# chahuja/mix-stage

Hardware: AMD Instinct MI355X
Metric: train-step clips/sec (B=32, T=64, M=8) (higher is better)
Workload: dtype f32; 1 GPU; Mix-StAGE GAN train step (reference D/G coin flip, seed 4321: 457 G + 510 D steps), B=32 clips per GPU, T=64, 128-mel, 104-dim pose, M=S=8, audio branch pinned; fp32 arithmetic (the reference trains in fp64, trainer.py:138; held to it at 1e-4 pose L1); global_batch=32, parallelism=dp1, hip_graphs=True, bn_sync=local

## Files before the change

### include/mixstage_aux.h

```cpp
#ifndef MIXSTAGE_AUX_H_
#define MIXSTAGE_AUX_H_

#include "mixstage.h"

#ifdef __cplusplus
extern "C" {
#endif

int ms_set_counter_buffer(int32_t* zeroed_counters, int n);

int ms_conv_block_bwd_overlap(const ms_conv_desc* d, const float* x, const float* x2, const float* w,
                              const float* gamma, const float* running_mean, const float* running_var,
                              const float* y_raw, const float* y, const float* save, const float* dy, float* dyr,
                              float* dx, float* dx2, float* dw, float* dbias, float* dgamma, float* dbeta,
                              void* workspace, size_t workspace_bytes, void* stream, void* side_stream,
                              void* side_workspace, size_t side_workspace_bytes);

int ms_timing_enable(int on);
size_t ms_timing_report(char* buf, size_t cap);

int ms_debug_set_patch_min_workgroups(int n);
int ms_debug_set_patch_tuning(int intra_split, int force_splitk);

int ms_debug_set_conv16_tile(int wm, int wn);
int ms_debug_set_conv16_ring(int nstg, int wide8);
int ms_debug_set_wgrad16_target(int workgroups);
int ms_debug_set_wgrad16_ring(int buffers);
int ms_debug_set_wgrad_target(int workgroups);
int ms_debug_set_wgrad_wave(int on);
int ms_debug_set_conv_tile(int on);
int ms_debug_set_bn_fused(int on);
int ms_debug_set_bn_fused_min_workgroups(int n);
int ms_debug_set_skip(const char* patterns);

int ms_debug_set_clip32(int on);

int ms_debug_set_clip_corun(int on);
int ms_debug_set_clip_corun_bwd(int on);

int ms_selftest_mfma(const float* A, const float* B, float* C, int K, void* stream);
int ms_probe_peak(int kind, long iters, void* a, void* b, double* work, void* stream);

#ifdef __cplusplus
}
#endif
#endif
```

### mix_stage_amd/_lib.py

```python
import ctypes
import os

_HERE = os.path.dirname(os.path.abspath(__file__))
LIB_PATH = os.path.join(_HERE, 'libmixstage_hip.so')
_ALT_LIB = os.environ.get('MS_LIB_PATH')
if _ALT_LIB:
  LIB_PATH = _ALT_LIB

c_void_p, c_int, c_float, c_size_t = ctypes.c_void_p, ctypes.c_int, ctypes.c_float, ctypes.c_size_t


class BwdOptions(ctypes.Structure):
  _fields_ = [('side_stream', ctypes.c_void_p), ('side_workspace', ctypes.c_void_p), ('side_workspace_bytes', ctypes.c_size_t),
              ('wt_prepared', ctypes.c_void_p), ('wgrad_partials', ctypes.c_void_p), ('defer_wgrad_launch', ctypes.c_int),
              ('prev_y', ctypes.c_void_p), ('prev_y_raw', ctypes.c_void_p), ('prev_save', ctypes.c_void_p), ('prev_gamma', ctypes.c_void_p),
              ('prev_dgamma', ctypes.c_void_p), ('prev_dbeta', ctypes.c_void_p), ('prev_dbias', ctypes.c_void_p), ('prev_slope', ctypes.c_float),
              ('bn_sync', ctypes.c_void_p), ('bn_sync_words', ctypes.c_int32), ('dy_is_dyr', ctypes.c_int),
              ('dx_accum', ctypes.c_void_p)]


class LossScale(ctypes.Structure):
  _fields_ = [('scale', ctypes.c_float), ('scale_dev', ctypes.c_void_p)]


# ... 142 lines not shown
    'ms_debug_set_patch_min_workgroups': (c_int, [c_int]),
    'ms_debug_set_patch_tuning': (c_int, [c_int, c_int]),
    'ms_debug_set_conv16_tile': (c_int, [c_int, c_int]),
    'ms_debug_set_conv16_ring': (c_int, [c_int, c_int]),
    'ms_debug_set_skip': (c_int, [ctypes.c_char_p]),
    'ms_debug_set_clip32': (c_int, [c_int]),
    'ms_debug_set_clip_corun': (c_int, [c_int]),
    'ms_clip_hold': (c_int, [_P]),
    'ms_clip_hold_flush': (c_int, [_P]),
    'ms_clip_hold_discard': (c_int, [_P]),
    'ms_clip_grid': (c_int, [_DESC]),
    'ms_clip_pair_ok': (c_int, [_DESC, _DESC]),
    'ms_clip_dgrad_grid': (c_int, [_DESC]),
    'ms_clip_dgrad_pair_ok': (c_int, [_DESC, _DESC]),
    'ms_debug_set_clip_corun_bwd': (c_int, [c_int]),
    'ms_debug_set_wgrad16_target': (c_int, [c_int]),
    'ms_debug_set_wgrad16_ring': (c_int, [c_int]),
    'ms_debug_set_wgrad_target': (c_int, [c_int]),
    'ms_debug_set_wgrad_wave': (c_int, [c_int]),
    'ms_debug_set_conv_tile': (c_int, [c_int]),
    'ms_set_wgrad_batched': (c_int, [c_int, c_int]),
    'ms_dgrad_fuses_prev_bn': (c_int, [_P]),
    'ms_dgrad_takes_accum': (c_int, [_P]),
    'ms_stat_pair_ok': (c_int, [_P]),
    'ms_selftest_mfma': (c_int, [_P, _P, _P, c_int, _P]),
    'ms_probe_peak': (c_int, [c_int, ctypes.c_long, _P, _P, ctypes.POINTER(ctypes.c_double), _P]),
}

_lib = None

# ... 42 lines not shown
```

### mix_stage_amd/csrc/api.hip

```cpp
#include "block_geom.h"

namespace ms {
extern int g_clip32;

static int validate(const ms_conv_desc* d, const char* who) {
  if (!d) return set_error("%s: null descriptor", who);
  if (d->B < 1 || d->Cin < 1 || d->Cout < 1 || d->groups < 1 || d->H < 1 || d->W < 1 || d->KH < 1 || d->KW < 1 ||
      d->SH < 1 || d->SW < 1 || d->PH < 0 || d->PW < 0)
    return set_error("%s: bad geometry", who);
  const int oh = (d->H + 2 * d->PH - d->KH) / d->SH + 1, ow = (d->W + 2 * d->PW - d->KW) / d->SW + 1;
  if (d->H + 2 * d->PH < d->KH || d->W + 2 * d->PW < d->KW || oh != d->OH || ow != d->OW)
    return set_error("%s: output size (%d,%d) does not match geometry (expected %d,%d)", who, d->OH, d->OW, oh, ow);
  if (d->mode < MS_BARE || d->mode > MS_BN_EVAL) return set_error("%s: bad mode %d", who, d->mode);
  if (d->in_mode < MS_IN_PLAIN || d->in_mode > MS_IN_UP2ADD) return set_error("%s: bad in_mode %d", who, d->in_mode);
  if (d->in_mode == MS_IN_UP2ADD && (d->H != 1 || d->KH != 1 || (d->W & 1)))
    return set_error("%s: UP2ADD needs a 1-D block with even W", who);
  if (dt_of(d) > DT_F16 || (d->dtype & ~(0xff | MS_DT_OUT_F32 | MS_DT_BN_FOLDED | MS_DT_STAT_PAIR | MS_DT_BN_FROZEN))) return set_error("%s: bad dtype 0x%x", who, d->dtype);
  if (dt_of(d) == DT_F32 && (d->dtype & ~(0xff | MS_DT_STAT_PAIR | MS_DT_BN_FROZEN))) return set_error("%s: MS_DT_OUT_F32 is a flag of the 16-bit modes", who);
  if ((d->dtype & MS_DT_BN_FROZEN) && d->mode != MS_BN_EVAL) return set_error("%s: MS_DT_BN_FROZEN is a flag of BN_EVAL blocks", who);
  if ((d->dtype & MS_DT_STAT_PAIR) && (d->B & 1)) return set_error("%s: MS_DT_STAT_PAIR needs an even batch", who);
  const double out_elems = (double)d->B * d->groups * d->Cout * d->OH * d->OW;
  const double in_elems = (double)d->B * d->groups * d->Cin * d->H * d->W;
  const double lim = dt_of(d) == DT_F32 ? 536870912.0 : 1073741824.0;
  if (out_elems >= lim || in_elems >= lim) return set_error("%s: tensor of 2 GiB or more (%.0f elements)", who, std::max(out_elems, in_elems));
// ... 742 lines not shown
}
int ms_clip_dgrad_pair_ok(const ms_conv_desc* host, const ms_conv_desc* guest) {
  if (validate(host, "ms_clip_dgrad_pair_ok") || validate(guest, "ms_clip_dgrad_pair_ok") || dt_of(host) != DT_F32 || dt_of(guest) != DT_F32 || g_precision != 0) return 0;
  return clip32_dgrad_pair_ok(host, guest) ? 1 : 0;
}
int ms_debug_set_clip_corun(int on) {
  const int prev = g_clip_corun < 0 ? 1 : g_clip_corun;
  g_clip_corun = on ? 1 : 0;
  return prev;
}
int ms_debug_set_clip_corun_bwd(int on) {
  const int prev = g_clip_corun_bwd < 0 ? 1 : g_clip_corun_bwd;
  g_clip_corun_bwd = on ? 1 : 0;
  return prev;
}

}
```

### mix_stage_amd/csrc/clip32.hip

```cpp
#include <stdio.h>
#include <stdlib.h>

#include <algorithm>
#include <map>
#include <mutex>
#include <vector>

#include "kernels.h"
#include "conv16.h"
#include "job_queue.h"

namespace ms {

typedef unsigned int cl_u32x4 __attribute__((ext_vector_type(4)));
typedef unsigned int cl_u32x2 __attribute__((ext_vector_type(2)));
constexpr int CL_SPIN_LIMIT = 1 << 21;
constexpr int CL_MAXK8W = 9;

struct Clip32Args {
  const float* x;
  const float* x2;
  const float* wp;
  const float* bias;
  const float* gamma;
// ... 721 lines not shown
    case 8: return clip32_launch_k<KW, S, NB, UP2, 8, DG2>(a, nwg, lds_bytes, s);
    case 9: return clip32_launch_k<KW, S, NB, UP2, 9, DG2>(a, nwg, lds_bytes, s);
    default: return clip32_launch_k<KW, S, NB, UP2, 0, DG2>(a, nwg, lds_bytes, s);
  }
}

struct ClipJob {
  Clip32Args a;
  int KW, S, nb, nwg, lds;
  bool up2, dg2;
  bool bwd;
  const char* what;
  double flops, bytes;
};

enum { CLIP_HOST_DOWN8 = 0, CLIP_HOST_UP8 = 1, CLIP_HOSTS = 2 };
enum { CLIP_GUEST_K3_4 = 0, CLIP_GUEST_DOWN2 = 1, CLIP_GUEST_DOWN4 = 2, CLIP_GUEST_DOWN8 = 3, CLIP_GUESTS = 4 };
enum { CLIP_BHOST_UP8 = 0, CLIP_BHOST_DOWN8 = 1 };
enum { CLIP_BGUEST_DG0 = 0, CLIP_BGUEST_DG2 = 1, CLIP_BGUEST_DG4 = 2, CLIP_BGUEST_DG8 = 3 };
static int clip_host_kind(const ClipJob& j) {
  if (j.a.k8w != 8) return -1;
  if (j.bwd) {
    if (j.up2) return -1;
    return j.dg2 ? CLIP_BHOST_DOWN8 : (j.KW == 3 && j.S == 1) ? CLIP_BHOST_UP8 : -1;
  }
  if (j.dg2) return -1;
  if (j.KW == 4 && j.S == 2 && !j.up2) return CLIP_HOST_DOWN8;
  if (j.KW == 3 && j.S == 1 && j.up2) return CLIP_HOST_UP8;
  return -1;
}
static int clip_guest_kind(const ClipJob& j) {
  if (j.up2) return -1;
  if (j.bwd) {
    if (!j.dg2) return -1;
    return j.a.k8w == 2 ? CLIP_BGUEST_DG2 : j.a.k8w == 4 ? CLIP_BGUEST_DG4 : j.a.k8w == 8 ? CLIP_BGUEST_DG8 : j.a.k8w == 9 ? -1 : CLIP_BGUEST_DG0;
  }
  if (j.dg2) return -1;
  if (j.KW == 3 && j.S == 1) return j.a.k8w == 4 ? CLIP_GUEST_K3_4 : -1;
  if (j.KW == 4 && j.S == 2) return j.a.k8w == 2 ? CLIP_GUEST_DOWN2 : j.a.k8w == 4 ? CLIP_GUEST_DOWN4 : j.a.k8w == 8 ? CLIP_GUEST_DOWN8 : -1;
  return -1;
}
static bool clip_pair_instance(const ClipJob& A, const ClipJob& B) {
  const int h = clip_host_kind(A), g = clip_guest_kind(B);
  if (h < 0 || g < 0 || A.bwd != B.bwd) return false;
  if (!A.bwd) return true;
  return h == CLIP_BHOST_UP8 ? (g == CLIP_BGUEST_DG0 || g == CLIP_BGUEST_DG8) : g != CLIP_BGUEST_DG0;
}
template <int KWA, int SA, int NBA, bool UP2A, int K8WA, int KWB, int SB, int NBB, bool UP2B, int K8WB, bool DG2A = false, bool DG2B = false>
static int clip32_pair_launch_k(const ClipPairArgs& pp, int nwg, int lds_bytes, hipStream_t s) {
  auto fn = clip32_pair_kernel<KWA, SA, NBA, UP2A, K8WA, KWB, SB, NBB, UP2B, K8WB, DG2A, DG2B>;
  static unsigned long long attr_done = 0;
  if (first_time_on_device(attr_done)) {
    if (hipFuncSetAttribute(reinterpret_cast<const void*>(fn), hipFuncAttributeMaxDynamicSharedMemorySize, 160 * 1024) != hipSuccess)
      return set_error("clip32: cannot raise the dynamic LDS limit");
    done_on_device(attr_done);
  }
  hipLaunchKernelGGL(fn, dim3(nwg), dim3(256), lds_bytes, s, pp);
  return check_launch("clip32_pair_kernel");
}
template <int KWA, int SA, int NBA, bool UP2A>
static int clip32_pair_launch_g(int guest, const ClipPairArgs& pp, int nwg, int lds_bytes, hipStream_t s) {
  switch (guest) {
    case CLIP_GUEST_K3_4: return clip32_pair_launch_k<KWA, SA, NBA, UP2A, 8, 3, 1, 2, false, 4>(pp, nwg, lds_bytes, s);
    case CLIP_GUEST_DOWN2: return clip32_pair_launch_k<KWA, SA, NBA, UP2A, 8, 4, 2, 1, false, 2>(pp, nwg, lds_bytes, s);
    case CLIP_GUEST_DOWN4: return clip32_pair_launch_k<KWA, SA, NBA, UP2A, 8, 4, 2, 1, false, 4>(pp, nwg, lds_bytes, s);
    default: return clip32_pair_launch_k<KWA, SA, NBA, UP2A, 8, 4, 2, 1, false, 8>(pp, nwg, lds_bytes, s);
  }
}
static int clip32_pair_launch_bwd(int host, int guest, const ClipPairArgs& pp, int nwg, int lds_bytes, hipStream_t s) {
  if (host == CLIP_BHOST_UP8) {
    if (guest == CLIP_BGUEST_DG0) return clip32_pair_launch_k<3, 1, 2, false, 8, 4, 1, 2, false, 0, false, true>(pp, nwg, lds_bytes, s);
    return clip32_pair_launch_k<3, 1, 2, false, 8, 4, 1, 2, false, 8, false, true>(pp, nwg, lds_bytes, s);
  }
  switch (guest) {
    case CLIP_BGUEST_DG2: return clip32_pair_launch_k<4, 1, 2, false, 8, 4, 1, 2, false, 2, true, true>(pp, nwg, lds_bytes, s);
    case CLIP_BGUEST_DG4: return clip32_pair_launch_k<4, 1, 2, false, 8, 4, 1, 2, false, 4, true, true>(pp, nwg, lds_bytes, s);
    default: return clip32_pair_launch_k<4, 1, 2, false, 8, 4, 1, 2, false, 8, true, true>(pp, nwg, lds_bytes, s);
  }
}

static int clip32_issue(ClipJob& j, hipStream_t s) {
  Clip32Args& a = j.a;
  const int nwg = j.nwg;
  TimingScope ts(s, j.flops, j.bytes, "clip32_kernel<%d,%d,%d,%d>|conv_%s_clip k1x%d s%d rows%d red%d T%d B%d ep%d", j.KW, j.S, j.nb, j.up2 ? 1 : 0, j.what,
// ... 21 lines not shown
      for (int k = 0; k < 8; ++k) {
        std::vector<double> v;
        for (int i = 0; i < nwg; ++i) if (h[(size_t)i * 8 + k]) v.push_back((double)(h[(size_t)i * 8 + k] - t0) * 0.01);
        if (v.empty()) continue;
        std::sort(v.begin(), v.end());
        fprintf(stderr, "  stamp %d: %7.2f %7.2f %7.2f\n", k, v.front(), v[v.size() / 2], v.back());
      }
    }
    a.stamps = nullptr;
  }
  return rc;
}

int g_clip_corun = -1;
int g_clip_corun_bwd = -1;
enum { HOLD_IDLE = 0, HOLD_ARMED = 1, HOLD_PENDING = 2 };
struct ClipHold {
  int state = HOLD_IDLE;
  ClipJob job;
  const char* ws_lo = nullptr;
  const char* ws_hi = nullptr;
};
static std::mutex g_hold_mu;
static std::map<hipStream_t, ClipHold> g_hold;
static thread_local bool t_in_call = false;
static thread_local const char* t_ws_lo = nullptr;
static thread_local const char* t_ws_hi = nullptr;

static bool clip_corun_on() {
  if (g_clip_corun < 0) { const char* e = getenv("MS_CLIP_CORUN"); g_clip_corun = e ? (atoi(e) != 0) : 1; }
  return g_clip_corun != 0;
}
static bool clip_corun_bwd_on() {
  if (g_clip_corun_bwd < 0) { const char* e = getenv("MS_CLIP_CORUN_BWD"); g_clip_corun_bwd = e ? (atoi(e) != 0) : 1; }
  return g_clip_corun_bwd != 0;
}

int clip32_hold_arm(hipStream_t s) {
  std::lock_guard<std::mutex> lk(g_hold_mu);
  ClipHold& h = g_hold[s];
  if (h.state == HOLD_PENDING) return set_error("ms_clip_hold: a held block is pending on this stream (flush or discard it first)");
  h.state = HOLD_ARMED;
  return 0;
}
void clip32_hold_discard(hipStream_t s) {
  std::lock_guard<std::mutex> lk(g_hold_mu);
  auto it = g_hold.find(s);
  if (it != g_hold.end()) it->second.state = HOLD_IDLE;
}
int clip32_hold_flush(hipStream_t s) {
  ClipJob job;
  {
// ... 41 lines not shown
  if (meetA && meetB && (A.a.part == B.a.part || A.a.sync == B.a.sync)) return false;
  return true;
}
static int clip32_issue_pair(ClipJob& A, ClipJob& B, hipStream_t s) {
  char da[96], db[96];
  snprintf(da, sizeof(da), "conv_%s_clip k1x%d s%d rows%d red%d T%d B%d ep%d", A.what, A.KW, A.S, A.a.rows_valid, A.a.Cin, A.a.To, A.a.B, A.a.ep);
  snprintf(db, sizeof(db), "conv_%s_clip k1x%d s%d rows%d red%d T%d B%d ep%d", B.what, B.KW, B.S, B.a.rows_valid, B.a.Cin, B.a.To, B.a.B, B.a.ep);
  TimingScope ts(s, A.flops + B.flops, A.bytes + B.bytes, "clip32_kernel<%d,%d,%d,%d>+<%d,%d,%d,%d>|%s + %s", A.KW, A.S, A.nb, A.up2 ? 1 : 0, B.KW, B.S,
                 B.nb, B.up2 ? 1 : 0, da, db);
  if (ts.skip()) return 0;
  ClipPairArgs pp;
  pp.nA = A.nwg; pp.a = A.a; pp.b = B.a;
  pp.a.stamps = pp.b.stamps = nullptr;
  const int nwg = A.nwg + B.nwg, lds = std::max(A.lds, B.lds), guest = clip_guest_kind(B);
  if (A.bwd) return clip32_pair_launch_bwd(clip_host_kind(A), guest, pp, nwg, lds, s);
  return clip_host_kind(A) == CLIP_HOST_DOWN8 ? clip32_pair_launch_g<4, 2, 1, false>(guest, pp, nwg, lds, s)
                                              : clip32_pair_launch_g<3, 1, 2, true>(guest, pp, nwg, lds, s);
}

int clip32_launch(Clip32Args a, int KW, int S, bool up2, const char* what, hipStream_t s, bool dg2 = false, ClipJob* plan = nullptr,
                  bool bwd = false) {
  const int nb = (S == 2 && !dg2) ? 1 : 2, npx = 32 * nb;
  a.k8w = clip_k8w(a.Cin);
  a.npw = a.B * a.To / npx;
  if (a.sg < 1) a.sg = 1;
  if (a.npw % a.sg) return -2;
  const int nct = cdiv(a.Cout, 32);
  a.nct = nct;
  const int ncl = npx / a.To, pslots = cl_pslots(ncl * (a.Ti + 2));
  const int img = 4 * a.k8w * 2 * pslots * 16, red = (4 * 32 * (npx + 4) + 4) * 4;
// ... 140 lines not shown
```

### mix_stage_amd/csrc/kernels.h

```cpp
#pragma once
#include <type_traits>

#include "common.h"

namespace ms {

enum { EP_BARE = 0, EP_LRELU = 1, EP_BN_EVAL = 2, EP_RAW_STATS = 3, EP_DGRAD = 4, EP_DGRAD_UP2 = 5, EP_BN_FUSED = 6, EP_DGRAD_BN = 7, EP_DGRAD_ACC = 8 };

struct GatherArgs {
  const float* A;
  const float* src;
  const float* src2;
  float* out;
  float* out2;
  const float* bias;
  const float* bn_g;
  const float* bn_b;
  const float* bn_m;
  const float* bn_v;
  float* stats;
  int Mg, Kg, groups, Kc, src_ctotal, SRCH, SRCW, OUTH, OUTW, Npix;
  int KH, KW, SH, SW, PH, PW;
  int bcast, a_vec, ep;
  int batch;
// ... 138 lines not shown
size_t clip32_fwd_weight_bytes(const ms_conv_desc* d);
size_t clip32_dgrad_weight_floats(const ms_conv_desc* d);
size_t clip32_weight_floats(int rows, int red, int KW);
int clip32_prep_queue(const float* w, float* out, int rows, int red, int KW, int transposed, int w_cols, hipStream_t s);
int clip32_prep_flush(hipStream_t s);
void clip32_prep_discard();
void gdgrad32_prep_discard();
struct PrepQueueGuard { ~PrepQueueGuard() { clip32_prep_discard(); gdgrad32_prep_discard(); } };
size_t clip32_part_bytes(int rows, int npw);
int clip32_sync_words(int rows);
int clip32_block_fwd(const ms_conv_desc* d, const float* x, const float* x2, const float* wp, const float* bias, const float* gamma,
                     const float* beta, float* rm, float* rv, float* y_raw, float* y, float* save, float* part, int* sync,
                     int sync_words, hipStream_t s);
extern int g_clip_corun;
extern int g_clip_corun_bwd;
int clip32_dgrad_grid(const ms_conv_desc* d);
bool clip32_dgrad_pair_ok(const ms_conv_desc* host, const ms_conv_desc* guest);
int clip32_hold_arm(hipStream_t s);
int clip32_hold_flush(hipStream_t s);
void clip32_hold_discard(hipStream_t s);
int clip32_call_begin(hipStream_t s, bool clip_path, const void* ws, size_t ws_bytes);
void clip32_call_end(hipStream_t s);
int clip32_fwd_grid(const ms_conv_desc* d);
bool clip32_fwd_pair_ok(const ms_conv_desc* host, const ms_conv_desc* guest);
struct Clip32PrevBN { const float* y; const float* y_raw; const float* save; const float* gamma; float* dgamma; float* dbeta; float* dbias; float slope; };
size_t clip32_dgrad_bn_part_bytes(const ms_conv_desc* d);
bool clip32_dgrad_bn_ok(const ms_conv_desc* d);
int clip32_block_dgrad(const ms_conv_desc* d, const float* g, const float* wp, float* dx, float* dx2, hipStream_t s,
                       const Clip32PrevBN* pv = nullptr, float* part = nullptr, int* sync = nullptr, int sync_words = 0,
                       const float* accum = nullptr);
// ... 98 lines not shown
```

### mix_stage_amd/gan.py

```python
import contextlib
import os

import torch
import torch.nn as nn

from . import ops, ops16


class ConstantLambdaScheduler:

  def __init__(self, lmbdas, **kwargs):
    self.lmbdas = list(lmbdas)

  def step(self):
    return list(self.lmbdas)

  def state(self):
    return ()

  def set_state(self, state):
    pass


class IncrementalLambdaScheduler:
# ... 107 lines not shown
      ops.check(ops.lib().ms_write_floats(ops._ptr(dev), vals, 2, ops._stream()), 'ms_write_floats')
    self._lambdas_written = now
    return dev

  def _score(self, pose):
    dt = getattr(self.D, '_ms_dt', 0)
    if dt and hasattr(self.D, 'forward_channel_major'):
      return self.D.forward_channel_major(ops16.btc_to_cb8(pose, dt, velocity=True))[0]
    v = ops.velocity_cm(pose)
    if hasattr(self.D, 'forward_channel_major'):
      return self.D.forward_channel_major(v)[0]
    return self.D(ops.to_time_major(v))[0]

  def _score_pair(self, first, second):
    D = self.D
    if not hasattr(D, 'forward_pair') or first.shape != second.shape or first.dtype != second.dtype or first.dim() != 3:
      return None
    if first.dtype != torch.float32 or not first.is_cuda:
      return None
    B, T, P = first.shape
    probe = self._pair_probe.get((B, T, P, first.device))
    if probe is None:
      probe = self._pair_probe[(B, T, P, first.device)] = torch.empty(2 * B, P, T, device='meta')
    if not D.pair_supported(probe):
      return None
    both = torch.cat([first, second], dim=0)
    dt = getattr(D, '_ms_dt', 0)
    return D.forward_pair(ops16.btc_to_cb8(both, dt, velocity=True) if dt else ops.velocity_cm(both), split=False)

  def forward(self, x_audio, y_pose, **kwargs):
    internal_losses = []
    if 'confidence' in kwargs and not (isinstance(kwargs['confidence'], (int, float)) and kwargs['confidence'] == 1):
      raise NotImplementedError('confidence weighting is not on the Mix-StAGE path (confidence == 1)')
    W, outputs = self.estimate_weights(x_audio, y_pose, **kwargs)
    if self.update_D_prob_flag:
      self.update_D_prob(W)

    if self.training:
      self.lambda_D, self.lambda_gan = self.lambda_scheduler.step()
      lam = None
      if y_pose.is_cuda:
        lam = self.write_lambdas(y_pose.device) if self._lambda_host_writes else self.lambda_device(y_pose.device)
      lam_D = lam[0] if lam is not None else self.lambda_D
      lam_gan = lam[1] if lam is not None else self.lambda_gan
      if torch.rand(1).item() < self.D_prob:
        self.G.eval()
        with torch.no_grad():
          fake_pose, partial_i_loss, *args = self.G(x_audio, y_pose, **kwargs)
          args = args[0] if len(args) > 0 else {}
        self.G.train(self.training)
        self.fake_flag = True
        pair = self._score_pair(fake_pose.detach(), y_pose) if self.pair_D_passes else None
        if pair is not None:
          if pair.dtype == torch.float32 and pair.numel() // 2 <= ops.LP_PAIR_MAX:
            fake_D_loss, real_D_loss = ops.lp_mean_pair(pair, (0.0, 1.0), (lam_D, 1.0), squared=self.criterion_name == 'MSELoss')
          else:
            fake_pose_score, real_pose_score = ops.split_halves(pair)
            fake_D_loss = self._loss(fake_pose_score, target=0.0, scale=lam_D)
            real_D_loss = self._loss(real_pose_score, target=1.0)
        else:
          fake_pose_score = self._score(fake_pose.detach())
          fake_D_loss = self._loss(fake_pose_score, target=0.0, scale=lam_D)
          real_pose_score = self._score(y_pose)
          real_D_loss = self._loss(real_pose_score, target=1.0)
        internal_losses.append(real_D_loss)
        internal_losses.append(fake_D_loss)
        internal_losses += partial_i_loss
        self.G_flag = False
      else:
        fake_pose, partial_i_loss, *args = self.G(x_audio, y_pose, **kwargs)
        args = args[0] if len(args) > 0 else {}
        if self.no_grad:
          with torch.no_grad():
            fake_pose_score = self._score(fake_pose)
        elif self.skip_D_weight_grads_in_G_step:
          with self._frozen_D():
            fake_pose_score = self._score(fake_pose)
        else:
          fake_pose_score = self._score(fake_pose)
        G_gan_loss = self._loss(fake_pose_score, target=1.0, scale=lam_gan)
        pose_loss = self._loss(fake_pose, y_pose)
        internal_losses.append(pose_loss)
        internal_losses.append(G_gan_loss)
        internal_losses += partial_i_loss
        self.G_flag = True
    else:
      fake_pose, partial_i_loss, *args = self.G(x_audio, y_pose, **kwargs)
# ... 10 lines not shown
```

### mix_stage_amd/joint_late_cluster_soft_style.py

```python
import contextlib

import torch
import torch.nn as nn

from . import ops, ops16
from .layers import (AudioEncoder, ClusterClassify, ConvNormRelu, Curriculum, EmbLin, Group, PoseEncoder,
                     PoseStyleEncoder, TextEncoder1D, UNet1D, bare_conv)
from .speech2gesture import Speech2Gesture_D

JointLateClusterSoftStyle4_D = Speech2Gesture_D


@contextlib.contextmanager
def some_grad(model):
  flags = [(p, p.requires_grad) for p in model.parameters()]
  for p, _ in flags:
    p.requires_grad_(False)
  try:
    yield
  finally:
    for p, f in flags:
      p.requires_grad_(f)


# ... 140 lines not shown
    if dt:
      x = ops16.to_cb8(x, dt)
    labels_score = self.classify_cluster(x)
    internal_losses.append(ops.cross_entropy(labels_score, labels, layout='bct'))

    chained = (ops16.decoder_chain16 if dt else ops.decoder_chain)(x, list(self.decoder), self.logits, labels_score, self.out_feats)
    if chained is not None:
      x, self.labels_cap_soft = chained
    else:
      z = self.decoder[0].forward_broadcast(x)
      for m in list(self.decoder)[1:]:
        z = m(z)
      z = bare_conv(self.logits, z, out_f32=True)
      x, self.labels_cap_soft = ops.softmax_mix(z, labels_score, self.out_feats)

    if pose_style_encoder_flag:
      if self.some_grad_flag:
        with some_grad(self.pose_style_encoder):
          pose_style_score_out = self.pose_style_encoder(x)
      else:
        pose_style_score_out = self.pose_style_encoder(x)
      id_out_loss = ops.cross_entropy(pose_style_score_out, style_id, scale=self.lambda_id)
    else:
      id_out_loss = torch.zeros(1)[0]

    internal_losses.append(id_in_loss if pose_style_encoder_flag else id_in_loss * self.lambda_id)
    internal_losses.append(id_out_loss if pose_style_encoder_flag else id_out_loss * self.lambda_id)
    return x, internal_losses
```

### mix_stage_amd/layers.py

```python
import torch
import torch.nn as nn

from . import ops, ops16
from ._lib import MS_BARE, MS_BN_EVAL, MS_BN_TRAIN, MS_IN_BCAST, MS_IN_PLAIN, MS_IN_UP2ADD, MS_LRELU


def set_compute_dtype(module, dtype):
  code = 0 if dtype in (None, 'fp32', 'f32', 'float32', torch.float32) else (
      ops16.MS_DT[dtype] if isinstance(dtype, torch.dtype) else ops16.NAME_DT[dtype])
  for m in module.modules():
    m._ms_dt = code
  return module


def set_inference_folding(module, on=True):
  for m in module.modules():
    if isinstance(m, ConvNormRelu):
      m._bn_folded = bool(on)
  return module


def compute_dtype(module):
  return getattr(module, '_ms_dt', 0)

# ... 76 lines not shown


def _default_padding(kernel_size, stride):
  kt, st = isinstance(kernel_size, tuple), isinstance(stride, tuple)
  if not kt and st:
    return tuple(int((kernel_size - s) / 2) for s in stride)
  if kt and not st:
    return tuple(int((k - stride) / 2) for k in kernel_size)
  if kt and st:
    assert len(kernel_size) == len(stride), \
        'dims in kernel_size are {} and stride are {}. They must be the same'.format(len(kernel_size), len(stride))
    return tuple(0 for _ in kernel_size)
  return int((kernel_size - stride) / 2)


def bare_conv(conv, x, lrelu_slope=None, out_f32=False):
  geom = getattr(conv, '_ms_geom', None)
  if geom is None:
    nd = 1 if isinstance(conv, nn.Conv1d) else 2
    geom = ops.ConvGeom(nd, conv.groups, conv.kernel_size, conv.stride, conv.padding,
                        slope=0.0 if lrelu_slope is None else lrelu_slope)
    conv._ms_geom = geom
  mode = MS_BARE if lrelu_slope is None else MS_LRELU
  dt = getattr(conv, '_ms_dt', 0)
  if dt:
    was_plain = not ops16.is_cb8(x)
    if was_plain:
      x = ops16.to_cb8(x, dt)
    y = ops16.conv_block16(x, conv.weight, conv.bias, geom, mode, out_f32=out_f32)
    return ops16.from_cb8(y, conv.weight.shape[0]) if (was_plain and not out_f32) else y
  return ops.conv_block(x, conv.weight, conv.bias, geom, mode)


class ConvNormRelu(nn.Module):
  def __init__(self, in_channels, out_channels, type='1d', leaky=False, downsample=False, kernel_size=None,
               stride=None, padding=None, p=0, groups=1):
    super(ConvNormRelu, self).__init__()
# ... 108 lines not shown
      return y if (was_plain or out_f32) else ops16.to_cb8(y, dt)
    return y

  def _next_desc(self, x):
    n = self.norm
    if self._nd != 1 or getattr(self, '_ms_dt', 0) or x.dim() != 3 or (self._p and self.training):
      return None
    frozen = bool(getattr(self, '_bn_frozen', False))
    train = self.training and n.track_running_stats and not frozen
    if train and ops.bn_sync_active():
      return None
    if frozen and torch.is_grad_enabled():
      return None
    w = self.conv.weight
    return self._geometry().desc(x.shape[0], w.shape[1], 1, x.shape[2], w.shape[0] // self.conv.groups, MS_BN_TRAIN if train else MS_BN_EVAL,
                                 MS_IN_PLAIN, 0)

  def forward(self, x, **kwargs):
    residual = kwargs.get('_residual')
    out_f32 = bool(kwargs.get('_out_f32'))
    if residual is not None:
      return self._run(x, x2=residual, in_mode=MS_IN_UP2ADD, out_f32=out_f32, link=kwargs.get('_ms_link'))
    if kwargs.get('_broadcast'):
      return self._run(x, in_mode=MS_IN_BCAST, out_f32=out_f32)
    return self._run(x, out_f32=out_f32, chain_prev=bool(kwargs.get('_ms_chain')), link=kwargs.get('_ms_link'))

  def forward_upsample_add(self, a, residual, _ms_link=None):
    return self(a, _residual=residual, _ms_link=_ms_link)

  def forward_broadcast(self, x):
    return self(x, _broadcast=True)
# ... 162 lines not shown
  def _score(x):
    x = x.mean(-1) if x.shape[-1] > 1 else x.squeeze(-1)
    return x.squeeze(dim=-1)

  def forward_beside(self, x, host, host_x):
    blocks = [m for m in list(host.modules()) + list(self.modules()) if isinstance(m, ConvNormRelu)]
    if (getattr(self, '_ms_dt', 0) or getattr(host, '_ms_dt', 0) or ops16.is_cb8(host_x) or not ops.corun_ok(x, host_x)
        or any(p.dtype != torch.float32 for p in self.parameters()) or _hooked(host, self, *blocks)
        or any(b._p and b.training for b in blocks)):
      out = host(host_x)
      return out, self(x)
    out, z = ops.corun(lambda: host(host_x), _chain_steps(self, x), x.device)
    return out, self._score(z)


class ClusterClassify(nn.Module):

  def __init__(self, num_clusters=8, kernel_size=None, stride=None, p=0, groups=1, input_channels=256):
    super().__init__()
    self.conv = nn.ModuleList()
    common = dict(type='1d', leaky=True, downsample=False, kernel_size=kernel_size, stride=stride, p=p, groups=groups)
    self.conv.append(ConvNormRelu(input_channels, 256, **common))
    self.conv += nn.ModuleList([ConvNormRelu(256, 256, **common) for i in range(5)])
    self.logits = nn.Conv1d(256 * groups, num_clusters * groups, kernel_size=1, stride=1, groups=groups)

  def forward(self, x, time_steps=None):
    dt = getattr(self, '_ms_dt', 0)
    if dt and not ops16.is_cb8(x):
      x = ops16.to_cb8(x, dt)
    for i, m in enumerate(self.conv):
# ... 70 lines not shown
```

### mix_stage_amd/ops.py

```python
import contextlib
import ctypes
import os

import torch

from . import _lib
from ._lib import (BwdOptions, ConvDesc, FwdOptions, MS_BARE, MS_BN_EVAL, MS_BN_TRAIN, MS_DT_STAT_PAIR, MS_IN_BCAST, MS_IN_PLAIN,
                   MS_IN_UP2ADD, MS_LRELU, check, lib)

_vp = ctypes.c_void_p


def _ptr(t):
  return None if t is None else _vp(t.data_ptr())


def _stream():
  return _vp(torch.cuda.current_stream().cuda_stream)


def _need_hip(*tensors):
  for t in tensors:
    if t is None:
      continue
# ... 8 lines not shown
_counters = {}
USE_IN_LAUNCH_SPLIT_REDUCTION = False


def _ensure_counters(device):
  key = (device.type, device.index)
  if key not in _counters:
    buf = torch.zeros(1 << 16, dtype=torch.int32, device=device)
    check(lib().ms_set_counter_buffer(_ptr(buf), buf.numel()), 'ms_set_counter_buffer')
    _counters[key] = buf
  return _counters[key]



_corun = {'driver': None, 'held': False, 'keep': [], 'on': os.environ.get('MS_CLIP_CORUN', '1') != '0', 'merges_offered': 0,
          'in_guest': False, 'bwd_on': os.environ.get('MS_CLIP_CORUN_BWD', '1') != '0', 'bwd_keep': [], 'bwd_offered': 0}


def workspace(nbytes, device):
  key = (device.type, device.index, torch.cuda.current_stream(device).cuda_stream)
  if _corun['held']:
    key = key + ('held',)
  if USE_IN_LAUNCH_SPLIT_REDUCTION:
    _ensure_counters(device)
  ws = _workspaces.get(key)
  if ws is None or ws.numel() < nbytes:
    size = max(int(nbytes * 1.5), 1 << 22)
    if ws is not None:
      _retired_workspaces.append(ws)
    ws = torch.empty(size, dtype=torch.uint8, device=device)
    _workspaces[key] = ws
# ... 326 lines not shown
    if pre is None:
      sync = None
      if mode == MS_BN_TRAIN and nd == 1:
        from . import ops16
        sync = ops16.block_sync(x.device, d)
      opt = FwdOptions(planes.data_ptr() if planes is not None else None, sync.data_ptr() if sync is not None else None,
                       sync.numel() if sync is not None else 0)
      check(lib().ms_conv_block_fwd_ex(ctypes.byref(d), _ptr(x), _ptr(x2), _ptr(w), _ptr(bias), _ptr(gamma), _ptr(beta),
                                       _ptr(rm), _ptr(rv), _ptr(y_raw), _ptr(y), _ptr(save), _ptr(ws), ws.numel(),
                                       _stream(), ctypes.byref(opt)), 'ms_conv_block_fwd_ex')
      if _corun['held']:
        _corun['keep'].append((x, x2, w, bias, gamma, beta, rm, rv, y_raw, y, save, ws, planes, sync))
    ctx.geom_desc = d
    ctx.mode, ctx.in_mode, ctx.frozen = mode, in_mode, frozen
    ctx.corun_guest = bool(_corun['in_guest'] and pre is None and not frozen and nd == 1 and xin is not None and xin.grad_fn is not None
                           and type(xin.grad_fn).__name__ == '_ConvBlockFnBackward'
                           and not (getattr(xin, '_backward_hooks', None) or getattr(xin, 'retains_grad', False)))
    ctx.prev = None
    ctx.dy_is_dyr = False
    if prev is not None and pre is None and in_mode == MS_IN_PLAIN and nd == 1 and getattr(prev, 'mode', None) == MS_BN_TRAIN \
        and not bn_sync_active() and lib().ms_dgrad_fuses_prev_bn(ctypes.byref(d)):
      from . import ops16
      py = prev.saved_tensors[5]
      watched = bool(getattr(x, '_backward_hooks', None)) or bool(getattr(x, 'retains_grad', False))
      if ops16.in_launch_meetings() and not watched and py is not None and py.data_ptr() == x.data_ptr() and tuple(py.shape) == tuple(x.shape):
        ctx.prev = prev
    ctx.link = None
    if link is not None and pre is None and nd == 1 and not bn_sync_active():
      lk, role = link
      if role == 'consumer' and in_mode == MS_IN_PLAIN and x.requires_grad and lib().ms_dgrad_takes_accum(ctypes.byref(d)) \
          and not (getattr(x, '_backward_hooks', None) or getattr(x, 'retains_grad', False)):
# ... 269 lines not shown
  try:
    drv = _CoRun(guest_steps, device)
    _corun['driver'] = drv
    try:
      out = host_fn()
    finally:
      _corun['driver'] = None
    return out, drv.finish()
  except BaseException:
    _corun['driver'] = None
    lib().ms_clip_hold_discard(_stream())
    _corun['keep'].clear()
    raise


def corun_ok(*tensors):
  from . import ops16
  return bool(_corun['on'] and _corun['driver'] is None and not bn_sync_active() and not _stat_pair['on'] and ops16.in_launch_meetings()
              and lib().ms_get_precision() == 0 and all(t.is_cuda and t.dtype == torch.float32 for t in tensors))


def enable_corun(on):
  old = _corun['on']
  _corun['on'] = bool(on)
  return old


def _bwd_guest_ok(d, dy):
  from . import ops16
  return bool(_corun['on'] and _corun['bwd_on'] and _corun['driver'] is None and not bn_sync_active() and not _stat_pair['on']
# ... 612 lines not shown

class _VelocityFn(torch.autograd.Function):
  @staticmethod
  def forward(ctx, x):
    _need_hip(x)
    x = x.contiguous()
    B, T, P = x.shape
    v = torch.empty((B, P, T), dtype=torch.float32, device=x.device)
    check(lib().ms_velocity_fwd(_ptr(x), _ptr(v), B, T, P, _stream()), 'ms_velocity_fwd')
    ctx.dims = (B, T, P)
    return v

  @staticmethod
  def backward(ctx, dv):
    B, T, P = ctx.dims
    dv = dv.contiguous()
    dx = torch.empty((B, T, P), dtype=torch.float32, device=dv.device)
    check(lib().ms_velocity_bwd(_ptr(dv), _ptr(dx), B, T, P, _stream()), 'ms_velocity_bwd')
    return dx


@_bridge64
def velocity_cm(x):
  return _VelocityFn.apply(x)


class _TransposeFn(torch.autograd.Function):
  @staticmethod
  def forward(ctx, x, to_cm):
    _need_hip(x)
# ... 245 lines not shown
```

### mix_stage_amd/speech2gesture.py

```python
import torch
import torch.nn as nn

from . import ops, ops16
from .layers import ConvNormRelu, bare_conv


class Speech2Gesture_D(nn.Module):

  def __init__(self, in_channels=104, out_channels=64, n_downsampling=2, p=0, groups=1, **kwargs):
    super(Speech2Gesture_D, self).__init__()
    self.conv1 = nn.Sequential(torch.nn.Conv1d(in_channels * groups, out_channels * groups, 4, 2, padding=1,
                                               groups=groups),
                               torch.nn.LeakyReLU(negative_slope=0.2))
    self.conv2 = nn.ModuleList([])
    for n in range(1, n_downsampling):
      ch_mul = min(2 ** n, 8)
      self.conv2.append(ConvNormRelu(out_channels, out_channels * ch_mul, type='1d', downsample=True, leaky=True,
                                     p=p, groups=groups))
    self.conv2 = nn.Sequential(*self.conv2)
    ch_mul_new = min(2 ** n_downsampling, 8)
    self.conv3 = ConvNormRelu(out_channels * ch_mul, out_channels * ch_mul_new, type='1d', leaky=True, kernel_size=4,
                              stride=1, p=p, groups=groups)
    out_shape = 1 if 'out_shape' not in kwargs else kwargs['out_shape']
    self.logits = nn.Conv1d(out_channels * ch_mul_new * groups, out_shape * groups, kernel_size=4, stride=1,
# ... 29 lines not shown
          break
        geom = mod._geometry() if mod is not None else ops.ConvGeom(1, conv.groups, conv.kernel_size, conv.stride, conv.padding)
        if W + 2 * geom.PW < geom.KW:
          ok = False
          break
        flags = (dt | (MS_DT_OUT_F32 if conv is self.logits else 0)) if dt else 0
        ok, W = ops.stat_pair_ok(geom, x.shape[0], conv.weight.shape[1], W, conv.weight.shape[0] // conv.groups, mode, flags)
      cache[key] = bool(ok)
    return cache[key]

  def forward_pair(self, x, split=True):
    with ops.stat_pair():
      s = self.forward_channel_major(x)[0]
    return ops.split_halves(s) if split else s

  def forward(self, x):
    dt = getattr(self, '_ms_dt', 0)
    if dt:
      return self.forward_channel_major(ops16.btc_to_cb8(x, dt))
    return self.forward_channel_major(ops.to_channel_major(x))
```

Measured before the change: 11450 clips/s.

## Co-run discriminator scoring alongside G's pose-style encoder via paired clip kernels

Adds a 'rider' mechanism so that, during the G step, the discriminator's channel-major forward runs as a guest alongside the pose-style encoder host in fused co-run clip kernels. New host kinds (DOWN2 forward, DOWN2 and K3 backward) and their pair launch instantiations let these smaller-width convolutions share one launch. It is on by default; the D-step variant stays off behind an env flag. The aim is to fill an under-occupied GPU with two small conv chains at once. The cost is extra template instantiations and more complex control flow, with possible numeric or ordering risks.

```diff
diff --git a/include/mixstage_aux.h b/include/mixstage_aux.h
--- a/include/mixstage_aux.h
+++ b/include/mixstage_aux.h
@@ -37,6 +37,7 @@
 
 int ms_debug_set_clip_corun(int on);
 int ms_debug_set_clip_corun_bwd(int on);
+int ms_debug_set_clip_corun_d(int on);
 
 int ms_selftest_mfma(const float* A, const float* B, float* C, int K, void* stream);
 int ms_probe_peak(int kind, long iters, void* a, void* b, double* work, void* stream);
diff --git a/mix_stage_amd/_lib.py b/mix_stage_amd/_lib.py
--- a/mix_stage_amd/_lib.py
+++ b/mix_stage_amd/_lib.py
@@ -180,6 +180,7 @@
     'ms_clip_dgrad_grid': (c_int, [_DESC]),
     'ms_clip_dgrad_pair_ok': (c_int, [_DESC, _DESC]),
     'ms_debug_set_clip_corun_bwd': (c_int, [c_int]),
+    'ms_debug_set_clip_corun_d': (c_int, [c_int]),
     'ms_debug_set_wgrad16_target': (c_int, [c_int]),
     'ms_debug_set_wgrad16_ring': (c_int, [c_int]),
     'ms_debug_set_wgrad_target': (c_int, [c_int]),
diff --git a/mix_stage_amd/csrc/api.hip b/mix_stage_amd/csrc/api.hip
--- a/mix_stage_amd/csrc/api.hip
+++ b/mix_stage_amd/csrc/api.hip
@@ -780,5 +780,10 @@
   g_clip_corun_bwd = on ? 1 : 0;
   return prev;
 }
-
-}
+int ms_debug_set_clip_corun_d(int on) {
+  const int prev = g_clip_corun_d < 0 ? 1 : g_clip_corun_d;
+  g_clip_corun_d = on ? 1 : 0;
+  return prev;
+}
+
+}
diff --git a/mix_stage_amd/csrc/clip32.hip b/mix_stage_amd/csrc/clip32.hip
--- a/mix_stage_amd/csrc/clip32.hip
+++ b/mix_stage_amd/csrc/clip32.hip
@@ -759,11 +759,15 @@
   double flops, bytes;
 };
 
-enum { CLIP_HOST_DOWN8 = 0, CLIP_HOST_UP8 = 1, CLIP_HOSTS = 2 };
+enum { CLIP_HOST_DOWN8 = 0, CLIP_HOST_UP8 = 1, CLIP_HOST_DOWN2 = 2, CLIP_HOSTS = 3 };
 enum { CLIP_GUEST_K3_4 = 0, CLIP_GUEST_DOWN2 = 1, CLIP_GUEST_DOWN4 = 2, CLIP_GUEST_DOWN8 = 3, CLIP_GUESTS = 4 };
-enum { CLIP_BHOST_UP8 = 0, CLIP_BHOST_DOWN8 = 1 };
+enum { CLIP_BHOST_UP8 = 0, CLIP_BHOST_DOWN8 = 1, CLIP_BHOST_DOWN2 = 2, CLIP_BHOST_K3_2 = 3 };
 enum { CLIP_BGUEST_DG0 = 0, CLIP_BGUEST_DG2 = 1, CLIP_BGUEST_DG4 = 2, CLIP_BGUEST_DG8 = 3 };
 static int clip_host_kind(const ClipJob& j) {
+  if (j.a.k8w == 2 && !j.up2) {
+    if (j.bwd) return j.dg2 ? CLIP_BHOST_DOWN2 : (j.KW == 3 && j.S == 1) ? CLIP_BHOST_K3_2 : -1;
+    return (!j.dg2 && j.KW == 4 && j.S == 2) ? CLIP_HOST_DOWN2 : -1;
+  }
   if (j.a.k8w != 8) return -1;
   if (j.bwd) {
     if (j.up2) return -1;
@@ -785,10 +789,13 @@
   if (j.KW == 4 && j.S == 2) return j.a.k8w == 2 ? CLIP_GUEST_DOWN2 : j.a.k8w == 4 ? CLIP_GUEST_DOWN4 : j.a.k8w == 8 ? CLIP_GUEST_DOWN8 : -1;
   return -1;
 }
+static bool clip_corun_d_on();
 static bool clip_pair_instance(const ClipJob& A, const ClipJob& B) {
   const int h = clip_host_kind(A), g = clip_guest_kind(B);
   if (h < 0 || g < 0 || A.bwd != B.bwd) return false;
-  if (!A.bwd) return true;
+  if (!A.bwd) return h != CLIP_HOST_DOWN2 || (clip_corun_d_on() && (g == CLIP_GUEST_DOWN2 || g == CLIP_GUEST_DOWN4));
+  if (h == CLIP_BHOST_DOWN2) return clip_corun_d_on() && g == CLIP_BGUEST_DG4;
+  if (h == CLIP_BHOST_K3_2) return clip_corun_d_on() && g == CLIP_BGUEST_DG2;
   return h == CLIP_BHOST_UP8 ? (g == CLIP_BGUEST_DG0 || g == CLIP_BGUEST_DG8) : g != CLIP_BGUEST_DG0;
 }
 template <int KWA, int SA, int NBA, bool UP2A, int K8WA, int KWB, int SB, int NBB, bool UP2B, int K8WB, bool DG2A = false, bool DG2B = false>
@@ -812,7 +819,13 @@
     default: return clip32_pair_launch_k<KWA, SA, NBA, UP2A, 8, 4, 2, 1, false, 8>(pp, nwg, lds_bytes, s);
   }
 }
+static int clip32_pair_launch_d(int guest, const ClipPairArgs& pp, int nwg, int lds_bytes, hipStream_t s) {
+  if (guest == CLIP_GUEST_DOWN4) return clip32_pair_launch_k<4, 2, 1, false, 2, 4, 2, 1, false, 4>(pp, nwg, lds_bytes, s);
+  return clip32_pair_launch_k<4, 2, 1, false, 2, 4, 2, 1, false, 2>(pp, nwg, lds_bytes, s);
+}
 static int clip32_pair_launch_bwd(int host, int guest, const ClipPairArgs& pp, int nwg, int lds_bytes, hipStream_t s) {
+  if (host == CLIP_BHOST_DOWN2) return clip32_pair_launch_k<4, 1, 2, false, 2, 4, 1, 2, false, 4, true, true>(pp, nwg, lds_bytes, s);
+  if (host == CLIP_BHOST_K3_2) return clip32_pair_launch_k<3, 1, 2, false, 2, 4, 1, 2, false, 2, false, true>(pp, nwg, lds_bytes, s);
   if (host == CLIP_BHOST_UP8) {
     if (guest == CLIP_BGUEST_DG0) return clip32_pair_launch_k<3, 1, 2, false, 8, 4, 1, 2, false, 0, false, true>(pp, nwg, lds_bytes, s);
     return clip32_pair_launch_k<3, 1, 2, false, 8, 4, 1, 2, false, 8, false, true>(pp, nwg, lds_bytes, s);
@@ -864,6 +877,7 @@
 
 int g_clip_corun = -1;
 int g_clip_corun_bwd = -1;
+int g_clip_corun_d = -1;
 enum { HOLD_IDLE = 0, HOLD_ARMED = 1, HOLD_PENDING = 2 };
 struct ClipHold {
   int state = HOLD_IDLE;
@@ -886,6 +900,11 @@
   return g_clip_corun_bwd != 0;
 }
 
+static bool clip_corun_d_on() {
+  if (g_clip_corun_d < 0) { const char* e = getenv("MS_CLIP_CORUN_D"); g_clip_corun_d = e ? (atoi(e) != 0) : 1; }
+  return g_clip_corun_d != 0;
+}
+
 int clip32_hold_arm(hipStream_t s) {
   std::lock_guard<std::mutex> lk(g_hold_mu);
   ClipHold& h = g_hold[s];
@@ -957,6 +976,7 @@
   pp.a.stamps = pp.b.stamps = nullptr;
   const int nwg = A.nwg + B.nwg, lds = std::max(A.lds, B.lds), guest = clip_guest_kind(B);
   if (A.bwd) return clip32_pair_launch_bwd(clip_host_kind(A), guest, pp, nwg, lds, s);
+  if (clip_host_kind(A) == CLIP_HOST_DOWN2) return clip32_pair_launch_d(guest, pp, nwg, lds, s);
   return clip_host_kind(A) == CLIP_HOST_DOWN8 ? clip32_pair_launch_g<4, 2, 1, false>(guest, pp, nwg, lds, s)
                                               : clip32_pair_launch_g<3, 1, 2, true>(guest, pp, nwg, lds, s);
 }
diff --git a/mix_stage_amd/csrc/kernels.h b/mix_stage_amd/csrc/kernels.h
--- a/mix_stage_amd/csrc/kernels.h
+++ b/mix_stage_amd/csrc/kernels.h
@@ -176,6 +176,7 @@
                      int sync_words, hipStream_t s);
 extern int g_clip_corun;
 extern int g_clip_corun_bwd;
+extern int g_clip_corun_d;
 int clip32_dgrad_grid(const ms_conv_desc* d);
 bool clip32_dgrad_pair_ok(const ms_conv_desc* host, const ms_conv_desc* guest);
 int clip32_hold_arm(hipStream_t s);
diff --git a/mix_stage_amd/gan.py b/mix_stage_amd/gan.py
--- a/mix_stage_amd/gan.py
+++ b/mix_stage_amd/gan.py
@@ -145,19 +145,51 @@
 
   def _score_pair(self, first, second):
     D = self.D
+    if not self._pair_ok(first, second):
+      return None
+    both = torch.cat([first, second], dim=0)
+    dt = getattr(D, '_ms_dt', 0)
+    return D.forward_pair(ops16.btc_to_cb8(both, dt, velocity=True) if dt else ops.velocity_cm(both), split=False)
+
+  def _pair_ok(self, first, second):
+    D = self.D
     if not hasattr(D, 'forward_pair') or first.shape != second.shape or first.dtype != second.dtype or first.dim() != 3:
-      return None
+      return False
     if first.dtype != torch.float32 or not first.is_cuda:
-      return None
+      return False
     B, T, P = first.shape
     probe = self._pair_probe.get((B, T, P, first.device))
     if probe is None:
       probe = self._pair_probe[(B, T, P, first.device)] = torch.empty(2 * B, P, T, device='meta')
-    if not D.pair_supported(probe):
+    return bool(D.pair_supported(probe))
+
+  def _rider(self, y_pose, d_step):
+    D = self.D
+    if not ops.corun_d_ok() or not hasattr(D, 'channel_major_steps') or getattr(D, '_ms_dt', 0) or not isinstance(y_pose, torch.Tensor):
       return None
-    both = torch.cat([first, second], dim=0)
-    dt = getattr(D, '_ms_dt', 0)
-    return D.forward_pair(ops16.btc_to_cb8(both, dt, velocity=True) if dt else ops.velocity_cm(both), split=False)
+    if d_step and not ops._corun['d_dstep']:
+      return None
+    if d_step:
+      def steps(pose):
+        first = pose.detach()
+        if not self.pair_D_passes or not self._pair_ok(first, y_pose):
+          return None
+        return D.channel_major_steps(lambda: ops.velocity_cm(torch.cat([first, y_pose], dim=0)), pair=True, around=torch.enable_grad)
+    else:
+      def steps(pose):
+        if pose.dim() != 3 or pose.dtype != torch.float32 or not pose.is_cuda:
+          return None
+        return D.channel_major_steps(lambda: ops.velocity_cm(pose), around=self._frozen_D)
+    return ops.Rider(steps)
+
+  def _run_G(self, rider, x_audio, y_pose, **kwargs):
+    if rider is None:
+      return self.G(x_audio, y_pose, **kwargs)
+    ops.set_rider((rider, self.D))
+    try:
+      return self.G(x_audio, y_pose, **kwargs)
+    finally:
+      ops.set_rider(None)
 
   def forward(self, x_audio, y_pose, **kwargs):
     internal_losses = []
@@ -176,12 +208,16 @@
       lam_gan = lam[1] if lam is not None else self.lambda_gan
       if torch.rand(1).item() < self.D_prob:
         self.G.eval()
+        rider = self._rider(y_pose, True) if self.pair_D_passes else None
         with torch.no_grad():
-          fake_pose, partial_i_loss, *args = self.G(x_audio, y_pose, **kwargs)
+          fake_pose, partial_i_loss, *args = self._run_G(rider, x_audio, y_pose, **kwargs)
           args = args[0] if len(args) > 0 else {}
         self.G.train(self.training)
         self.fake_flag = True
-        pair = self._score_pair(fake_pose.detach(), y_pose) if self.pair_D_passes else None
+        if rider is not None and rider.ran:
+          pair = rider.result
+        else:
+          pair = self._score_pair(fake_pose.detach(), y_pose) if self.pair_D_passes else None
         if pair is not None:
           if pair.dtype == torch.float32 and pair.numel() // 2 <= ops.LP_PAIR_MAX:
             fake_D_loss, real_D_loss = ops.lp_mean_pair(pair, (0.0, 1.0), (lam_D, 1.0), squared=self.criterion_name == 'MSELoss')
@@ -199,9 +235,12 @@
         internal_losses += partial_i_loss
         self.G_flag = False
       else:
-        fake_pose, partial_i_loss, *args = self.G(x_audio, y_pose, **kwargs)
+        rider = self._rider(y_pose, False) if (not self.no_grad and self.skip_D_weight_grads_in_G_step) else None
+        fake_pose, partial_i_loss, *args = self._run_G(rider, x_audio, y_pose, **kwargs)
         args = args[0] if len(args) > 0 else {}
-        if self.no_grad:
+        if rider is not None and rider.ran:
+          fake_pose_score = rider.result
+        elif self.no_grad:
           with torch.no_grad():
             fake_pose_score = self._score(fake_pose)
         elif self.skip_D_weight_grads_in_G_step:
diff --git a/mix_stage_amd/joint_late_cluster_soft_style.py b/mix_stage_amd/joint_late_cluster_soft_style.py
--- a/mix_stage_amd/joint_late_cluster_soft_style.py
+++ b/mix_stage_amd/joint_late_cluster_soft_style.py
@@ -178,12 +178,17 @@
       z = bare_conv(self.logits, z, out_f32=True)
       x, self.labels_cap_soft = ops.softmax_mix(z, labels_score, self.out_feats)
 
+    rider = ops.take_rider()
     if pose_style_encoder_flag:
+      if rider is not None and not dt and isinstance(x, torch.Tensor):
+        second_pass = lambda: self.pose_style_encoder.forward_carrying(x, rider[0], rider[1])
+      else:
+        second_pass = lambda: self.pose_style_encoder(x)
       if self.some_grad_flag:
         with some_grad(self.pose_style_encoder):
-          pose_style_score_out = self.pose_style_encoder(x)
+          pose_style_score_out = second_pass()
       else:
-        pose_style_score_out = self.pose_style_encoder(x)
+        pose_style_score_out = second_pass()
       id_out_loss = ops.cross_entropy(pose_style_score_out, style_id, scale=self.lambda_id)
     else:
       id_out_loss = torch.zeros(1)[0]
diff --git a/mix_stage_amd/layers.py b/mix_stage_amd/layers.py
--- a/mix_stage_amd/layers.py
+++ b/mix_stage_amd/layers.py
@@ -114,13 +114,18 @@
   return int((kernel_size - stride) / 2)
 
 
-def bare_conv(conv, x, lrelu_slope=None, out_f32=False):
+def bare_conv_geom(conv, lrelu_slope=None):
   geom = getattr(conv, '_ms_geom', None)
   if geom is None:
     nd = 1 if isinstance(conv, nn.Conv1d) else 2
     geom = ops.ConvGeom(nd, conv.groups, conv.kernel_size, conv.stride, conv.padding,
                         slope=0.0 if lrelu_slope is None else lrelu_slope)
     conv._ms_geom = geom
+  return geom
+
+
+def bare_conv(conv, x, lrelu_slope=None, out_f32=False):
+  geom = bare_conv_geom(conv, lrelu_slope)
   mode = MS_BARE if lrelu_slope is None else MS_LRELU
   dt = getattr(conv, '_ms_dt', 0)
   if dt:
@@ -259,7 +264,7 @@
       return None
     w = self.conv.weight
     return self._geometry().desc(x.shape[0], w.shape[1], 1, x.shape[2], w.shape[0] // self.conv.groups, MS_BN_TRAIN if train else MS_BN_EVAL,
-                                 MS_IN_PLAIN, 0)
+                                 MS_IN_PLAIN, ops.MS_DT_STAT_PAIR if ops.stat_pair_active() else 0)
 
   def forward(self, x, **kwargs):
     residual = kwargs.get('_residual')
@@ -452,6 +457,29 @@
     return out, self._score(z)
 
 
+  def forward_carrying(self, x, rider, other):
+    mods = [m for m in list(self.modules()) + list(other.modules())]
+    blocks = [m for m in mods if isinstance(m, ConvNormRelu)]
+    if (not ops.corun_d_ok() or getattr(self, '_ms_dt', 0) or getattr(other, '_ms_dt', 0) or not ops.corun_ok(x)
+        or any(p.dtype != torch.float32 for p in list(self.parameters()) + list(other.parameters())) or _hooked(*mods)
+        or any(b._p and b.training for b in blocks)):
+      return self(x)
+    steps = rider.steps(x)
+    if steps is None:
+      return self(x)
+    xc = ops.to_channel_major(x)
+
+    def host():
+      z = xc
+      for i, m in enumerate(self.conv):
+        z = m(z, _ms_chain=_chain_ok(self.conv, i))
+      return self._score(z)
+    out, rider.result = ops.corun(host, steps, x.device)
+    rider.ran = True
+    ops._corun['riders_run'] += 1
+    return out
+
+
 class ClusterClassify(nn.Module):
 
   def __init__(self, num_clusters=8, kernel_size=None, stride=None, p=0, groups=1, input_channels=256):
diff --git a/mix_stage_amd/ops.py b/mix_stage_amd/ops.py
--- a/mix_stage_amd/ops.py
+++ b/mix_stage_amd/ops.py
@@ -46,7 +46,9 @@
 
 
 _corun = {'driver': None, 'held': False, 'keep': [], 'on': os.environ.get('MS_CLIP_CORUN', '1') != '0', 'merges_offered': 0,
-          'in_guest': False, 'bwd_on': os.environ.get('MS_CLIP_CORUN_BWD', '1') != '0', 'bwd_keep': [], 'bwd_offered': 0}
+          'in_guest': False, 'bwd_on': os.environ.get('MS_CLIP_CORUN_BWD', '1') != '0', 'bwd_keep': [], 'bwd_offered': 0,
+          'd_on': os.environ.get('MS_CLIP_CORUN_D', '1') != '0', 'd_dstep': os.environ.get('MS_CLIP_CORUN_D_DSTEP', '0') != '0',
+          'rider': None, 'riders_run': 0}
 
 
 def workspace(nbytes, device):
@@ -403,7 +405,7 @@
     ctx.geom_desc = d
     ctx.mode, ctx.in_mode, ctx.frozen = mode, in_mode, frozen
     ctx.corun_guest = bool(_corun['in_guest'] and pre is None and not frozen and nd == 1 and xin is not None and xin.grad_fn is not None
-                           and type(xin.grad_fn).__name__ == '_ConvBlockFnBackward'
+                           and not pair and type(xin.grad_fn).__name__ in ('_ConvBlockFnBackward', '_VelocityFnBackward')
                            and not (getattr(xin, '_backward_hooks', None) or getattr(xin, 'retains_grad', False)))
     ctx.prev = None
     ctx.dy_is_dyr = False
@@ -703,6 +705,41 @@
     raise
 
 
+class Rider:
+  __slots__ = ('steps', 'ran', 'result')
+
+  def __init__(self, steps):
+    self.steps, self.ran, self.result = steps, False, None
+
+
+def set_rider(rider):
+  old = _corun['rider']
+  _corun['rider'] = rider
+  return old
+
+
+def take_rider():
+  rider, _corun['rider'] = _corun['rider'], None
+  return rider
+
+
+def corun_d_ok():
+  return bool(_corun['d_on'] and _corun['on'])
+
+
+def enable_corun_d(on):
+  old = _corun['d_on']
+  _corun['d_on'] = bool(on)
+  lib().ms_debug_set_clip_corun_d(1 if on else 0)
+  return old
+
+
+def enable_corun_d_dstep(on):
+  old = _corun['d_dstep']
+  _corun['d_dstep'] = bool(on)
+  return old
+
+
 def corun_ok(*tensors):
   from . import ops16
   return bool(_corun['on'] and _corun['driver'] is None and not bn_sync_active() and not _stat_pair['on'] and ops16.in_launch_meetings()
@@ -1345,6 +1382,8 @@
   @staticmethod
   def backward(ctx, dv):
     B, T, P = ctx.dims
+    if _corun['bwd_keep']:
+      _bwd_hold_release()
     dv = dv.contiguous()
     dx = torch.empty((B, T, P), dtype=torch.float32, device=dv.device)
     check(lib().ms_velocity_bwd(_ptr(dv), _ptr(dx), B, T, P, _stream()), 'ms_velocity_bwd')
diff --git a/mix_stage_amd/speech2gesture.py b/mix_stage_amd/speech2gesture.py
--- a/mix_stage_amd/speech2gesture.py
+++ b/mix_stage_amd/speech2gesture.py
@@ -1,8 +1,10 @@
+import contextlib
+
 import torch
 import torch.nn as nn
 
 from . import ops, ops16
-from .layers import ConvNormRelu, bare_conv
+from .layers import ConvNormRelu, bare_conv, bare_conv_geom
 
 
 class Speech2Gesture_D(nn.Module):
@@ -67,6 +69,32 @@
       s = self.forward_channel_major(x)[0]
     return ops.split_halves(s) if split else s
 
+  def channel_major_steps(self, make_x, pair=False, around=None):
+    from ._lib import MS_IN_PLAIN, MS_LRELU
+
+    def run(fn, *args, **kw):
+      with (around() if around is not None else contextlib.nullcontext()):
+        if pair:
+          with ops.stat_pair():
+            return fn(*args, **kw)
+        return fn(*args, **kw)
+
+    def bare_desc(conv, x, slope):
+      bare_conv_geom(conv, slope)
+      return conv._ms_geom.desc(x.shape[0], conv.weight.shape[1], 1, x.shape[2], conv.weight.shape[0] // conv.groups, MS_LRELU, MS_IN_PLAIN,
+                                ops.MS_DT_STAT_PAIR if pair else 0)
+    x = run(make_x)
+    slope = self.conv1[1].negative_slope
+    yield bare_desc(self.conv1[0], x, slope) if x.dim() == 3 else None
+    x = run(bare_conv, self.conv1[0], x, lrelu_slope=slope)
+    for m in self.conv2:
+      yield run(m._next_desc, x)
+      x = run(m, x)
+    yield None
+    x = run(self.conv3, x)
+    yield None
+    return run(lambda: bare_conv(self.logits, x, out_f32=True).transpose(-1, -2).squeeze(dim=-1))
+
   def forward(self, x):
     dt = getattr(self, '_ms_dt', 0)
     if dt:
```

Result: no change. 11510 clips/s, median of 6 (+0.5%).
